# svohr/mixemt

Measured on AMD Instinct MI355X. Metric: read x hap cells/sec through the EM iteration (EM iters/sec reported beside it as em_iters_per_s), 1000000 reads x 5408 haps in total, whole job, higher is better.
Workload: dtype f64

## Files before the change

include/mixemt_hip_tuning.h:

```cpp
#ifndef MIXEMT_HIP_TUNING_H
#define MIXEMT_HIP_TUNING_H

#include <stddef.h>
#include <stdint.h>

#ifdef __cplusplus
extern "C" {
#endif

struct mxm_em_state;

int mxm_reset_tuning(void);

int mxm_set_timing_events(void *ev_start, void *ev_stop);

int mxm_describe_stream_kernel(int32_t H, int32_t nb, char *buf, size_t len);

int mxm_diag_stream_read(const void *src, size_t bytes, int32_t wg_per_cu, int32_t blocked,
                         void *sink, void *stream);

struct mxm_coded;
int mxm_diag_stream_coded(const struct mxm_coded *c, int32_t H, int32_t wg_per_cu, void *sink, void *stream);

int mxm_diag_stream_quads(const struct mxm_coded *c, int32_t H, int32_t wg_per_cu, void *sink, void *stream);

int mxm_set_progress_callback(void (*fn)(const struct mxm_em_state *state_host, int32_t B, void *user),
                              void *user, int32_t every);

int mxm_set_loop_graph(int32_t mode);

int mxm_set_loop_fused(int32_t mode, int32_t chunk);

int mxm_set_fused_coded_grid(int32_t nwg);

int mxm_set_quad_left_grid(int32_t nwg);

int mxm_set_sparse_long_rows(int32_t on);
int mxm_set_sparse_long_entries(int32_t n);

int mxm_set_quad_encoder(int32_t kind);

int mxm_set_coded_batch_tile(int32_t bt);

int mxm_diag_fused_force_abort(int32_t on);

int mxm_diag_fused_stamps(const void *ws, unsigned long long *out_host);

int mxm_set_batch_tile(int32_t bt);

int mxm_set_compact_restarts(int32_t mode);

#define MXM_SAMPLES_TILE_ROWS 32
int mxm_samples_tile_rows(void);

int mxm_set_min_rows_per_wg(int32_t n);

int mxm_set_sparse_max_distinct(int32_t n);

#ifdef __cplusplus
}
#endif
#endif
```

mixemt_amd/_lib.py:

```python

import ctypes
import os

_PKG = os.path.dirname(os.path.abspath(__file__))
LIB_PATH = os.environ.get("MXM_LIB") or os.path.join(_PKG, "lib", "libmixemt_hip.so")

c_i32, c_i64, c_f64 = ctypes.c_int32, ctypes.c_int64, ctypes.c_double
c_ptr, c_size = ctypes.c_void_p, ctypes.c_size_t


class EmState(ctypes.Structure):
    _fields_ = [("done", c_i32), ("iters", c_i32), ("l1", c_f64), ("ticket", ctypes.c_uint32), ("error", ctypes.c_uint32)]


class Coded(ctypes.Structure):
    _fields_ = [("rec", c_ptr), ("rec_off", c_ptr), ("ndist", c_ptr), ("R", c_i64),
                ("P_rest", c_ptr), ("ldp_rest", c_i64), ("w_rest", c_ptr), ("R_rest", c_i64),
                ("wide_rows", c_ptr), ("n_wide", c_i64),
                ("qrec", c_ptr), ("qoff", c_ptr), ("nquad", c_ptr), ("quad_rows", c_ptr), ("n_quad_rows", c_i64),
                ("byte_rows", c_ptr), ("n_byte_rows", c_i64)]


class SampleTile(ctypes.Structure):
    _fields_ = [("sample", c_i32), ("count", c_i32), ("first", c_i64)]
# ... 110 lines not shown
                                      ctypes.POINTER(c_ptr)]),
    "mxm_aln_sizes_of": (ctypes.c_int, [c_ptr, ctypes.POINTER(AlnSizes)]),
    "mxm_aln_fetch": (ctypes.c_int, [c_ptr, c_ptr, c_ptr, c_ptr, c_ptr, c_ptr, c_ptr, c_ptr, c_ptr, c_ptr]),
    "mxm_aln_fetch_fragments": (ctypes.c_int, [c_ptr, c_ptr, c_ptr, c_ptr, c_ptr]),
    "mxm_aln_free": (None, [c_ptr]),
    "mxm_bam_read": (ctypes.c_int, [ctypes.c_char_p, c_i32, ctypes.POINTER(c_ptr)]),
    "mxm_bam_sizes_of": (ctypes.c_int, [c_ptr, ctypes.POINTER(BamSizes)]),
    "mxm_bam_columns": (ctypes.c_int, [c_ptr, ctypes.POINTER(AlnColumns)]),
    "mxm_bam_fetch_names": (ctypes.c_int, [c_ptr, c_ptr, c_ptr, c_ptr, c_ptr]),
    "mxm_bam_free": (None, [c_ptr]),
    "mxm_observe_bases": (ctypes.c_int, [ctypes.POINTER(AlnColumns), c_ptr, c_i32, c_i32, c_i64, c_ptr, c_ptr]),
    "mxm_observe_bases_labelled": (ctypes.c_int, [ctypes.POINTER(AlnColumns), c_ptr, c_ptr, c_i32, c_i32, c_i32, c_i64,
                                                  c_ptr, c_ptr]),
    "mxm_consensus": (ctypes.c_int, [c_ptr, c_i32, c_i64, c_i64, c_i64, c_i32, c_ptr, c_ptr, c_ptr, c_ptr]),
    "mxm_new_variants": (ctypes.c_int, [c_ptr, c_i64, c_i32, ctypes.POINTER(c_i32), c_i32, c_i64, c_ptr, c_ptr, c_ptr]),
    "mxm_first_observed": (ctypes.c_int, [ctypes.POINTER(AlnColumns), c_ptr, c_ptr, c_i32, c_i32, c_i32, c_i64, c_ptr,
                                          c_ptr, c_ptr]),
    "mxm_extend_assign": (ctypes.c_int, [ctypes.POINTER(AlnColumns), c_ptr, c_ptr, c_i32, c_i32, ctypes.POINTER(c_i32),
                                         c_i32, c_i32, c_i32, c_i32, c_ptr, c_i64, c_ptr, c_ptr, c_ptr, c_ptr]),
    "mxm_set_compact_restarts": (ctypes.c_int, [c_i32]),
    "mxm_set_loop_graph": (ctypes.c_int, [c_i32]),
    "mxm_set_loop_fused": (ctypes.c_int, [c_i32, c_i32]),
    "mxm_set_progress_callback": (ctypes.c_int, [c_ptr, c_ptr, c_i32]),
    "mxm_set_min_rows_per_wg": (ctypes.c_int, [c_i32]),
    "mxm_reset_tuning": (ctypes.c_int, []),
    "mxm_describe_stream_kernel": (ctypes.c_int, [c_i32, c_i32, ctypes.c_char_p, c_size]),
    "mxm_set_sparse_max_distinct": (ctypes.c_int, [c_i32]),
    "mxm_row_argmax_votes": (ctypes.c_int, [c_ptr, c_i64, c_ptr, c_i64, c_i32, c_ptr, c_ptr,
                                            c_ptr, c_size, c_ptr]),
    "mxm_first_seen": (ctypes.c_int, [c_ptr, c_i64, c_i32, c_ptr, c_ptr]),
    "mxm_gather_columns": (ctypes.c_int, [c_ptr, c_i64, c_i64, c_i32, c_ptr, c_i32, c_ptr, c_i64, c_ptr]),
    "mxm_fold_logaddexp": (ctypes.c_int, [c_ptr, c_i64, ctypes.POINTER(c_ptr), ctypes.POINTER(c_i64), c_i32,
                                          c_i64, c_i32, c_f64, c_ptr]),
}

FINISH_SIGNATURES = {
    "mxm_samples_finish_workspace_bytes": (c_size, [c_i64, c_i32, c_i32]),
    "mxm_votes_samples": (ctypes.c_int, [ctypes.POINTER(Coded), c_ptr, c_i32, c_i32, c_ptr, c_ptr, c_ptr, c_ptr, c_ptr, c_ptr,
                                         c_ptr, c_ptr, c_ptr, c_ptr, c_ptr, c_size, c_ptr]),
    "mxm_gather_columns_samples": (ctypes.c_int, [ctypes.POINTER(Coded), c_ptr, c_i32, c_i32, c_ptr, c_ptr, c_i32, c_ptr,
                                                  c_ptr, c_size, c_ptr]),
    "mxm_em_loop_samples_narrow": (ctypes.c_int, [ctypes.POINTER(Coded), c_ptr, c_i32, c_i32, c_ptr, c_i32, c_ptr, c_ptr,
                                                  c_ptr, c_ptr, c_ptr, c_ptr, c_f64, c_i32, c_i32, c_ptr, c_ptr, c_size,
                                                  c_ptr, ctypes.POINTER(EmState)]),
    "mxm_assign_reads_samples": (ctypes.c_int, [ctypes.POINTER(Coded), c_ptr, c_i32, c_i32, c_ptr, c_i32, c_ptr, c_ptr,
                                                c_ptr, c_ptr, c_ptr, c_ptr, c_f64, c_ptr, c_ptr, c_ptr, c_size, c_ptr]),
}

VARCHECK_SIGNATURES = {
    "mxm_check_variants_samples": (ctypes.c_int, [c_ptr, c_i32, c_i64, c_ptr, c_ptr, c_i32, c_ptr, c_ptr, c_i32, c_i64, c_ptr,
                                                  c_ptr, c_i32, c_f64, c_f64, c_f64, c_i32, c_i32, c_ptr, c_ptr, c_ptr, c_ptr]),
}

ABI_VERSION = 603

PROGRESS_FN = ctypes.CFUNCTYPE(None, ctypes.POINTER(EmState), c_i32, c_ptr)

_lib = None


class MixemtHipError(RuntimeError):
    pass


def load():
    global _lib
    if _lib is not None:
        return _lib
    if not os.path.exists(LIB_PATH):
        raise MixemtHipError(
            "libmixemt_hip.so is not built (%s); run `python -m mixemt_amd.build` -- "
            "there is no CPU fallback for the EM hot path" % LIB_PATH)
    from . import _dev
    lib = ctypes.CDLL(LIB_PATH)
    try:
        lib.mxm_version.restype = ctypes.c_int
        lib.mxm_version.argtypes = []
        have = lib.mxm_version()
    except AttributeError:
        have = None
    if have != ABI_VERSION:
        raise MixemtHipError("%s reports ABI version %s, this binding was written for %d: rebuild with "
                             "`python -m mixemt_amd.build --force`" % (LIB_PATH, have, ABI_VERSION))
    for name, (restype, argtypes) in (list(SIGNATURES.items()) + list(FINISH_SIGNATURES.items())
                                      + list(VARCHECK_SIGNATURES.items())):
        try:
            fn = getattr(lib, name)
        except AttributeError:
            raise MixemtHipError("%s has ABI version %d but lacks %s: rebuild with "
                                 "`python -m mixemt_amd.build --force`" % (LIB_PATH, have, name))
        fn.restype = restype
        fn.argtypes = argtypes
    _lib = lib
    try:
        if _dev.torch is not None and _dev.torch.cuda.is_available():
            lib.mxm_preload()
    except Exception:
        pass
    return lib


def check(rc, what):
    if rc != 0:
        msg = load().mxm_last_error().decode("utf-8", "replace")
        raise ValueError("%s failed (%d): %s" % (what, rc, msg))
```

mixemt_amd/build.py:

```python

import hashlib
import os
import shutil
import subprocess
import sys

_PKG = os.path.dirname(os.path.abspath(__file__))
_ROOT = os.path.dirname(_PKG)
SRC = os.path.join(_PKG, "csrc", "mixemt_hip.hip")
HDRS = [os.path.join(_ROOT, "include", name) for name in ("mixemt_hip.h", "mixemt_hip_tuning.h", "mixemt_hip_samples_finish.h",
                                                           "mixemt_hip_var_check.h")]
LIB_DIR = os.path.join(_PKG, "lib")
LIB = os.path.join(LIB_DIR, "libmixemt_hip.so")
ARCH = "gfx950"


def _hipcc():
    for cand in (os.environ.get("HIPCC"), shutil.which("hipcc"), "/opt/rocm/bin/hipcc"):
        if cand and os.path.exists(cand):
            return cand
    raise RuntimeError("hipcc not found (set HIPCC or add /opt/rocm/bin to PATH)")


def _sources():
    csrc = os.path.dirname(SRC)
    return sorted(os.path.join(csrc, f) for f in os.listdir(csrc) if f.endswith((".hip", ".hpp"))) + HDRS


def _digest(flags):
    h = hashlib.sha256()
    for path in _sources():
        with open(path, "rb") as fin:
            h.update(fin.read())
    h.update(" ".join(flags).encode())
    return h.hexdigest()


def build(force=False, defines=(), verbose=False, out=None):
    global LIB
    if out is not None:
        LIB = os.path.abspath(out)
    flags = ["--offload-arch=%s" % ARCH, "-O3", "-std=c++17", "-shared", "-fPIC", "-Werror=format",
             "-I" + os.path.join(_ROOT, "include"), "-I" + os.path.dirname(SRC)]
    flags += ["-D%s" % d for d in defines]
    stamp = LIB + ".stamp"
    want = _digest(flags)
    if not force and os.path.exists(LIB) and os.path.exists(stamp):
        with open(stamp) as fin:
            if fin.read().strip() == want:
                return LIB
    os.makedirs(os.path.dirname(LIB), exist_ok=True)
    cmd = [_hipcc()] + flags + [SRC, "-o", LIB, "-lz"]
    if verbose:
        sys.stderr.write(" ".join(cmd) + "\n")
    proc = subprocess.run(cmd, stdout=subprocess.PIPE, stderr=subprocess.STDOUT, text=True)
    if proc.returncode != 0:
        raise RuntimeError("hipcc failed:\n" + proc.stdout)
    with open(stamp, "w") as fout:
        fout.write(want + "\n")
    return LIB


if __name__ == "__main__":
    defs = []
# ... 14 lines not shown
```

mixemt_amd/csrc/coded_kernels.hpp:

```cpp
#ifndef MIXEMT_CODED_KERNELS_HPP
#define MIXEMT_CODED_KERNELS_HPP

#define ENC_THREADS 256
#define ENC_SLOTS 1024
#define ENC_MAX_CODES 256
#define ENC_MAX_WIDE 1024
#define ENC_WIDE_SLOTS 4096
#define ENC_EMPTY 0xFFFFFFFFFFFFFFFFull

__host__ __device__ __forceinline__ int rec_code_bytes(int nd, int ldc) { return nd > ENC_MAX_CODES ? 2 * ldc : ldc; }
__device__ __forceinline__ int rec_code_at(const uint8_t *codes, int h, bool wide) {
    return wide ? (int)reinterpret_cast<const uint16_t *>(codes)[h] : (int)codes[h];
}

template <int NCH, bool WIDE>
__device__ __forceinline__ void encode_one_row(int64_t r, const double *__restrict__ M, int64_t ldm, int H, int ldc,
                                               uint8_t *__restrict__ rec, int64_t rec_cap, int64_t *__restrict__ rec_off,
                                               int32_t *__restrict__ ndist, double *__restrict__ rowmax,
                                               unsigned long long *__restrict__ stats) {
    constexpr int NW = ENC_THREADS / 64;
    constexpr int SLOTS = WIDE ? ENC_WIDE_SLOTS : ENC_SLOTS;
    constexpr int MAXC = WIDE ? ENC_MAX_WIDE : ENC_MAX_CODES;
    constexpr int SPT = SLOTS / ENC_THREADS;
    __shared__ unsigned long long s_key[SLOTS];
// ... 150 lines not shown
                } else {
                    reinterpret_cast<unsigned int *>(rec + off)[t + k * ENC_THREADS] =
                        cd[0] | (cd[1] << 8) | (cd[2] << 16) | (cd[3] << 24);
                }
            }
        }
    }
    if (t == 0) {
        if constexpr (WIDE) {
            if (off >= 0) {
                ndist[r] = D;
                rec_off[r] = off;
                atomicAdd(&stats[1], ~0ull);
            }
        } else {
            rowmax[r] = shift;
            ndist[r] = (off >= 0) ? D : 0;
            rec_off[r] = (off >= 0) ? off : 0;
            if (off < 0) atomicAdd(&stats[1], 1ull);
        }
    }
    __syncthreads();
}

template <int NCH>
__global__ __launch_bounds__(ENC_THREADS) void encode_rows_kernel(
    const double *__restrict__ M, int64_t ldm, int64_t R, int H, int ldc, uint8_t *__restrict__ rec, int64_t rec_cap,
    int64_t *__restrict__ rec_off, int32_t *__restrict__ ndist, double *__restrict__ rowmax,
    unsigned long long *__restrict__ stats) {
    for (int64_t r = blockIdx.x; r < R; r += gridDim.x)
        encode_one_row<NCH, false>(r, M, ldm, H, ldc, rec, rec_cap, rec_off, ndist, rowmax, stats);
}

template <int NCH>
__global__ __launch_bounds__(ENC_THREADS) void encode_wide_rows_kernel(
    const double *__restrict__ M, int64_t ldm, int64_t R, int H, int ldc, uint8_t *__restrict__ rec, int64_t rec_cap,
    int64_t *__restrict__ rec_off, int32_t *__restrict__ ndist, double *__restrict__ rowmax,
    unsigned long long *__restrict__ stats) {
    constexpr int CH = 32;
    __shared__ int s_list[CH];
    __shared__ int s_nlist;
    const int t = threadIdx.x;
    const int64_t nchunk = (R + CH - 1) / CH;
    for (int64_t c = blockIdx.x; c < nchunk; c += gridDim.x) {
        if (t == 0) s_nlist = 0;
        __syncthreads();
        const int64_t r = c * CH + t;
        if (t < CH && r < R && ndist[r] == 0) s_list[atomicAdd(&s_nlist, 1)] = t;
        __syncthreads();
        const int n = s_nlist;
        for (int i = 0; i < n; ++i)
            encode_one_row<NCH, true>(c * CH + s_list[i], M, ldm, H, ldc, rec, rec_cap, rec_off, ndist, rowmax, stats);
        __syncthreads();
    }
}

template <int THREADS, int NCH, int NBUF, bool NT, bool RESIDENT, bool WIDE_PREFETCH, bool CHECK = false>
__device__ __forceinline__ void coded_row_pass(const uint8_t *__restrict__ rec, const int64_t *__restrict__ rec_off,
                                               const int32_t *__restrict__ ndist, int ldc, const double *__restrict__ w,
                                               const int64_t *__restrict__ wide_rows, int64_t n_wide, int64_t R,
                                               const double (&p)[NCH][4], double (&acc)[NCH][4], bool &meta_ready,
                                               int *chk_result = nullptr, const int64_t *__restrict__ row_list = nullptr,
                                               int64_t n_list = 0, const int32_t *__restrict__ nquad = nullptr, int vbid = -1,
                                               int vgrid = 0) {
    static_assert(NBUF >= 3, "codes NBUF - 1 rows ahead, tables NBUF - 2");
    constexpr int NW = THREADS / 64;
    constexpr int AUX = NT ? 2 : 0;
    __shared__ double s_tbl[NBUF][ENC_MAX_CODES];
    __shared__ __attribute__((aligned(16))) double red[NBUF][NW];
    const int t = threadIdx.x, lane = t & 63, wv = t >> 6;
    const int nword = ldc >> 2;
    const int64_t bid = vbid >= 0 ? (int64_t)vbid : (int64_t)blockIdx.x, grid = vbid >= 0 ? (int64_t)vgrid : (int64_t)gridDim.x;
    const row_deal deal(row_list != nullptr ? n_list : R, bid, grid);
    const int voff = t * 4;
    int last_w = t + (NCH - 1) * THREADS;
    if (last_w > nword - 1) last_w = nword - 1;
    const int voff_last = last_w * 4;
    const bool tbl_thread = (THREADS <= ENC_MAX_CODES) || t < ENC_MAX_CODES;
    const int tslot = t & (ENC_MAX_CODES - 1);
    typedef unsigned int u2v __attribute__((ext_vector_type(2)));
    __shared__ int s_chk[2];
    if constexpr (CHECK) {
        if (t == 0) s_chk[0] = s_chk[1] = 0;
        __syncthreads();
    }
    auto list_row = [&](int64_t e) -> int64_t {
        int64_t r = wide_rows[e];
        if constexpr (CHECK) {
            if (r < 0 || r >= R || (e > 0 && wide_rows[e - 1] >= r)) {
                s_chk[1] = 1;
                r = -1;
            }
        }
        return r;
    };
    auto list_nd = [&](int64_t r) -> int {
        if (r < 0) return 0;
        int nd = ndist[r];
        if constexpr (CHECK) {
            if (nd <= ENC_MAX_CODES) {
                s_chk[1] = 1;
                nd = 0;
            }
        }
        return nd;
    };
// ... 443 lines not shown
```

mixemt_amd/csrc/mixemt_hip.hip:

```cpp
#include <hip/hip_runtime.h>
#include <stdint.h>
#include <stdio.h>
#include <stdlib.h>
#include <string.h>
#include <math.h>
#include <algorithm>
#include <atomic>
#include <mutex>
#include <type_traits>
#include <utility>
#include <vector>

#include "mixemt_hip.h"
#include "mixemt_hip_tuning.h"

#include "common.hpp"
#include "aln_encode.hpp"
#include "bam_reader.hpp"
#include "coded_kernels.hpp"
#include "quad_kernels.hpp"
#include "quad_batched_kernels.hpp"
#include "build_kernels.hpp"
#include "build_lut_kernels.hpp"
#include "build_sparse_kernels.hpp"
#include "em_kernels.hpp"
#include "estep_kernels.hpp"
#include "aux_kernels.hpp"
#include "records_kernels.hpp"
#include "fused_kernels.hpp"
#include "fused_cols_kernels.hpp"
#include "fused_coded_kernels.hpp"
#include "fused_narrow_kernels.hpp"
#include "samples_kernels.hpp"
#include "samples_finish_kernels.hpp"
#include "exchange.hpp"
#include "aln_walk.hpp"
#include "observe_kernels.hpp"
#include "var_check_kernels.hpp"
#include "assemble_kernels.hpp"


struct mxm_em_state;
typedef void (*mxm_progress_fn)(const mxm_em_state *state_host, int32_t B, void *user);
struct mxm_tuning {
    int sparse_maxd = -1;
    int min_rows_per_wg = 8;
    int compact_restarts = 2;
    int max_bt = 4;
    int loop_graph = -1;
    int loop_fused = -1;
    int fused_chunk = 0;
    int fused_cols = 1;
    int fused_coded_wg = 0;
    int quad_left_wg = 0;
    int sparse_long_entries = 5120;
    int quad_encoder = 1;
    int sparse_long = 1;
    int coded_bt = 3;
    int fused_force_abort = 0;
    double fused_cells = 1.0e8;
    hipEvent_t ev_start = nullptr, ev_stop = nullptr;
    mxm_progress_fn progress = nullptr;
    void *progress_user = nullptr;
    int progress_every = 10;
};
static std::mutex g_tune_mu;
static mxm_tuning g_tune;
static thread_local mxm_tuning T;
#define MXM_ENTER() do { std::lock_guard<std::mutex> lk_(g_tune_mu); T = g_tune; } while (0)
template <typename F>
static int tune_set(F f) {
    std::lock_guard<std::mutex> lk(g_tune_mu);
    f(g_tune);
    return 0;
}
extern "C" int mxm_reset_tuning(void) {
    return tune_set([](mxm_tuning &t) { t = mxm_tuning(); });
}

static inline int clamp_grid(int64_t want, int cap) {
    if (want < 1) want = 1;
    return (int)(want < cap ? want : cap);
}

static inline int64_t part_ld(int H) { return ((int64_t)H + 1) & ~(int64_t)1; }

static hipError_t raise_dynamic_lds(const void *kernel, size_t bytes, const char *name) {
    const hipError_t e = hipFuncSetAttribute(kernel, hipFuncAttributeMaxDynamicSharedMemorySize, (int)bytes);
    if (e != hipSuccess)
        snprintf(g_err, sizeof(g_err), "%s: cannot opt into %zu bytes of dynamic LDS: %s", name, bytes,
                 hipGetErrorString(e));
    return e;
}
static int dynamic_lds_ok(const void *kernel, size_t bytes, const char *name, const char *who = nullptr, int H = 0,
                          const char *too_wide = nullptr) {
    if (too_wide != nullptr && bytes > 150 * 1024) return fail(-1, "%s: H=%d %s", who, H, too_wide);
    if (bytes > 60 * 1024 && raise_dynamic_lds(kernel, bytes, name) != hipSuccess) return -2;
    return 0;
}

#define RC_TRY(expr)                                                                         \
    do {                                                                                     \
        const int rc_ = (expr);                                                              \
        if (rc_ != 0) return rc_;                                                            \
    } while (0)

template <int MAX, typename F>
static bool dispatch_width(int n, F &&f) {
    if constexpr (MAX < 1) {
// ... 286 lines not shown
extern "C" int mxm_linearize(const double *M, int64_t ldm, int64_t R, int32_t H, double *P, int64_t ldp,
                             double *rowmax, void *stream) {
    if (R < 0 || H <= 0) return fail(-1, "mxm_linearize: bad shape");
    if (ldm < H || ldp < H || (ldp & 1)) return fail(-1, "mxm_linearize: ldp must be even and >= H (ldp=%lld)", (long long)ldp);
    if (R == 0) return 0;
    if (wide_rows_ok(M, ldm, H) && (reinterpret_cast<uintptr_t>(P) & 15) == 0 &&
        linearize_wide<double>(M, ldm, R, (int)H, P, ldp, rowmax, (hipStream_t)stream) == 0) {
        HIP_TRY(hipGetLastError());
        return 0;
    }
    const int grid = clamp_grid(R, num_cu() * 8);
    hipLaunchKernelGGL(linearize_kernel, dim3(grid), dim3(ROW_THREADS), 0, (hipStream_t)stream, M, ldm, R,
                       (int)H, P, ldp, rowmax);
    HIP_TRY(hipGetLastError());
    return 0;
}

extern "C" int mxm_set_timing_events(void *ev_start, void *ev_stop) {
    return tune_set([=](mxm_tuning &t) { t.ev_start = (hipEvent_t)ev_start; t.ev_stop = (hipEvent_t)ev_stop; });
}

extern "C" int mxm_set_min_rows_per_wg(int32_t n) {
    if (n < 1) return fail(-1, "mxm_set_min_rows_per_wg: n < 1");
    return tune_set([n](mxm_tuning &t) { t.min_rows_per_wg = n; });
}

extern "C" int mxm_set_compact_restarts(int32_t mode) {
    return tune_set([mode](mxm_tuning &t) { t.compact_restarts = mode < 0 ? 0 : (mode > 2 ? 2 : mode); });
}

extern "C" int mxm_set_batch_tile(int32_t bt) {
    if (bt < 1 || bt > 4) return fail(-1, "mxm_set_batch_tile: tile must be 1..4");
    return tune_set([bt](mxm_tuning &t) { t.max_bt = bt; });
}

extern "C" int mxm_set_fused_coded_grid(int32_t nwg) {
    return tune_set([nwg](mxm_tuning &t) { t.fused_coded_wg = nwg > 0 ? nwg : 0; });
}

extern "C" int mxm_set_sparse_long_rows(int32_t on) {
    return tune_set([on](mxm_tuning &t) { t.sparse_long = on ? 1 : 0; });
}
extern "C" int mxm_set_sparse_long_entries(int32_t n) {
    return tune_set([n](mxm_tuning &t) { t.sparse_long_entries = n > 0 ? n : 0; });
}
extern "C" int mxm_set_coded_batch_tile(int32_t bt) {
    if (bt != 1 && bt != 3) return fail(-1, "mxm_set_coded_batch_tile: 1 or 3, got %d", bt);
    return tune_set([bt](mxm_tuning &t) { t.coded_bt = bt; });
}
extern "C" int mxm_set_quad_encoder(int32_t kind) {
    if (kind != 0 && kind != 1) return fail(-1, "mxm_set_quad_encoder: 0 or 1, got %d", kind);
    return tune_set([kind](mxm_tuning &t) { t.quad_encoder = kind; });
}
extern "C" int mxm_set_quad_left_grid(int32_t nwg) {
    return tune_set([nwg](mxm_tuning &t) { t.quad_left_wg = nwg > 0 ? nwg : 0; });
}

extern "C" int mxm_diag_fused_force_abort(int32_t on) {
    return tune_set([on](mxm_tuning &t) { t.fused_force_abort = on ? 1 : 0; });
}

#ifndef MXM_V1_THREADS
#define MXM_V1_THREADS 256
#endif
#ifndef MXM_V1_NBUF
#define MXM_V1_NBUF 2
#endif
#ifndef MXM_V1_WG_PER_CU
#define MXM_V1_WG_PER_CU 2
#endif
#ifndef MXM_V2_THREADS
#define MXM_V2_THREADS 512
#endif
#ifndef MXM_V2_NBUF
#define MXM_V2_NBUF 2
#endif
#ifndef MXM_V3_THREADS
#define MXM_V3_THREADS 512
#endif
#ifndef MXM_V3_NBUF
#define MXM_V3_NBUF 2
#endif
#ifndef MXM_V4_THREADS
#define MXM_V4_THREADS 512
#endif
#ifndef MXM_V4_NBUF
#define MXM_V4_NBUF 2
#endif
#ifndef MXM_V2_PREG
#define MXM_V2_PREG 1
#endif
#ifndef MXM_V3_PREG
#define MXM_V3_PREG 2
#endif
#ifndef MXM_V4_PREG
#define MXM_V4_PREG 2
#endif
#ifndef MXM_V1B_THREADS
#define MXM_V1B_THREADS 512
#endif
#ifndef MXM_V1B_NBUF
#define MXM_V1B_NBUF 3
#endif
#define MXM_MAX_COL2 4096
#define MXM_LDS_BUDGET (156 * 1024)

// ... 238 lines not shown
    for (int b = 0; b < B;) {
        const int left = B - b;
        const int passes = (left + max_bt - 1) / max_bt;
        const int nb = (left + passes - 1) / passes;
        const mxm_em_state *st = state ? state + b : nullptr;
        int rc;
        if (linear)
            rc = em_iter_linear_tile(P, ldp, w, props, R, (int)H, nb, slots_from(b), state, colsum, (double *)ws,
                                     (hipStream_t)stream, b == 0);
        else
            rc = em_iter_log_one(M, ldm, w, ln_props ? ln_props + (int64_t)b * H : nullptr, R, (int)H, st,
                                 colsum + (int64_t)b * H, (double *)ws, (hipStream_t)stream);
        if (rc != 0) return rc;
        b += nb;
    }
    return 0;
}

extern "C" int mxm_linearize_f32(const double *M, int64_t ldm, int64_t R, int32_t H, float *P, int64_t ldp,
                                 double *rowmax, void *stream) {
    if (R < 0 || H <= 0) return fail(-1, "mxm_linearize_f32: bad shape");
    if (ldm < H || ldp < H || (ldp & 3)) return fail(-1, "mxm_linearize_f32: ldp must be a multiple of 4 and >= H (ldp=%lld)", (long long)ldp);
    if (R == 0) return 0;
    if (wide_rows_ok(M, ldm, H) && (reinterpret_cast<uintptr_t>(P) & 7) == 0 && (ldp & 1) == 0 &&
        linearize_wide<float>(M, ldm, R, (int)H, P, ldp, rowmax, (hipStream_t)stream) == 0) {
        HIP_TRY(hipGetLastError());
        return 0;
    }
    const int grid = clamp_grid(R, num_cu() * 8);
    hipLaunchKernelGGL(linearize_f32_kernel, dim3(grid), dim3(ROW_THREADS), 0, (hipStream_t)stream, M, ldm, R, (int)H,
                       P, ldp, rowmax);
    HIP_TRY(hipGetLastError());
    return 0;
}

extern "C" int mxm_em_iter_f32(const float *P, int64_t ldp, const double *w, const double *props, int64_t R,
                               int32_t H, int32_t B, const mxm_em_state *state, double *colsum, void *ws,
                               size_t ws_bytes, void *stream) {
    MXM_ENTER();
    if (R <= 0 || H <= 0 || B <= 0) return fail(-1, "mxm_em_iter_f32: bad shape R=%lld H=%d", (long long)R, H);
    if (!mxm_linear_supported(H)) return fail(-1, "mxm_em_iter_f32: H=%d outside the linear kernel's range", H);
    if (P == nullptr || (ldp & 3) || ldp < H) return fail(-1, "mxm_em_iter_f32: ldp must be a multiple of 4 and >= H");
    if (ws == nullptr || ws_bytes < mxm_workspace_bytes(R, H, B)) return fail(-1, "mxm_em_iter_f32: workspace too small");
    for (int b = 0; b < B; ++b) {
        const int rc = em_iter_f32_one(P, ldp, w, props + (int64_t)b * H, R, (int)H, state ? state + b : nullptr,
                                       colsum + (int64_t)b * H, (double *)ws, (hipStream_t)stream, b == 0);
        if (rc != 0) return rc;
    }
    return 0;
}

extern "C" size_t mxm_coded_bytes(int64_t R, int32_t H) { return mxm_record_bytes(R, H); }

extern "C" int mxm_encode_rows(const double *M, int64_t ldm, int64_t R, int32_t H, uint8_t *rec, size_t rec_bytes,
                               int64_t *rec_off, int32_t *ndist, double *rowmax, int64_t *stats, void *stream) {
    if (R <= 0 || H <= 0 || ldm < H) return fail(-1, "mxm_encode_rows: bad shape R=%lld H=%d", (long long)R, H);
    if (!mxm_linear_supported(H) || (reinterpret_cast<uintptr_t>(M) & 7) != 0)
        return fail(-1, "mxm_encode_rows: needs H in [65, 8192] (H=%d ldm=%lld)", H, (long long)ldm);
    if (rec == nullptr || (reinterpret_cast<uintptr_t>(rec) & 15) || rec_bytes < (size_t)coded_ld(H) + 16 * ENC_MAX_CODES)
        return fail(-1, "mxm_encode_rows: record buffer missing, unaligned or smaller than one record");
    if (rec_off == nullptr || ndist == nullptr || rowmax == nullptr || stats == nullptr)
        return fail(-1, "mxm_encode_rows: output arrays required");
    hipStream_t s = (hipStream_t)stream;
    HIP_TRY(hipMemsetAsync(stats, 0, 2 * sizeof(int64_t), s));
    const int ldc = coded_ld(H);
    const int nch = (ldc / 4 + ENC_THREADS - 1) / ENC_THREADS;
    const int grid = clamp_grid(R, num_cu() * 4);
    const int grid_w = clamp_grid((R + 31) / 32, num_cu() * 3);
    const bool ok = dispatch_width<8>(nch, [&](auto n) {
        constexpr int NCH = decltype(n)::value;
        unsigned long long *st = reinterpret_cast<unsigned long long *>(stats);
        hipLaunchKernelGGL((encode_rows_kernel<NCH>), dim3(grid), dim3(ENC_THREADS), 0, s, M, ldm, R, (int)H, ldc, rec,
                           (int64_t)rec_bytes, rec_off, ndist, rowmax, st);
        hipLaunchKernelGGL((encode_wide_rows_kernel<NCH>), dim3(grid_w), dim3(ENC_THREADS), 0, s, M, ldm, R, (int)H, ldc, rec,
                           (int64_t)rec_bytes, rec_off, ndist, rowmax, st);
    });
    if (!ok) return fail(-1, "mxm_encode_rows: H=%d outside the kernel's range", H);
    HIP_TRY(hipGetLastError());
    return 0;
}

static int coded_check(const mxm_coded *c, int32_t H, const char *who) {
    if (c == nullptr || c->R <= 0 || H <= 0 || !mxm_linear_supported(H))
        return fail(-1, "%s: bad coded matrix (rows %lld, H %d)", who, (long long)(c ? c->R : 0), H);
    if (c->rec == nullptr || c->rec_off == nullptr || c->ndist == nullptr) return fail(-1, "%s: coded matrix arrays missing", who);
    if (c->R_rest < 0 || (c->R_rest > 0 && (c->P_rest == nullptr || c->ldp_rest < H || (c->ldp_rest & 1) ||
                                            (reinterpret_cast<uintptr_t>(c->P_rest) & 15))))
        return fail(-1, "%s: the dense rest needs 16-byte aligned rows with an even ld >= H", who);
    if (c->n_wide < 0 || (c->n_wide > 0 && c->wide_rows == nullptr)) return fail(-1, "%s: n_wide > 0 needs wide_rows", who);
    if (c->qrec != nullptr) {
        if (c->qoff == nullptr || c->nquad == nullptr || c->n_quad_rows < 0 || c->n_byte_rows < 0 ||
            (c->n_quad_rows > 0 && c->quad_rows == nullptr) || (c->n_byte_rows > 0 && c->byte_rows == nullptr) ||
            (reinterpret_cast<uintptr_t>(c->qrec) & 31))
            return fail(-1, "%s: quad dictionary arrays missing (or qrec not 32-byte aligned)", who);
        if (c->n_quad_rows + c->n_byte_rows + c->n_wide + c->R_rest != c->R)
            return fail(-1, "%s: quad_rows + byte_rows + wide_rows + the dense rest must be all %lld rows", who, (long long)c->R);
    }
    return 0;
}

static int rest_check(const char *who, int32_t H, const double *M_rest, int64_t ldm_rest, const int64_t *rest_rows, int64_t n_rest) {
    if (n_rest < 0 || (n_rest > 0 && (M_rest == nullptr || rest_rows == nullptr || ldm_rest < H)))
        return fail(-1, "%s: the rows without a record need M_rest, rest_rows and ldm_rest >= H", who);
    return 0;
}

extern "C" size_t mxm_quad_bytes(int64_t R, int32_t H) {
    (void)H;
    constexpr size_t largest = QUAD_CODE_BYTES + QUAD_MAX * 32, per_piece = (size_t)QUAD_CHUNK / largest;
    return R > 0 ? (((size_t)R + per_piece - 1) / per_piece + 5120) * (size_t)QUAD_CHUNK : 0;
}

extern "C" int mxm_expand_tables(const uint8_t *maj, const int32_t *mk_ptr, const uint16_t *mk_hap, const uint8_t *mk_base,
                                 const uint8_t *map256, int32_t S, int32_t H, int64_t lde, uint8_t *out, void *stream) {
    if (maj == nullptr || mk_ptr == nullptr || mk_hap == nullptr || mk_base == nullptr || out == nullptr || S <= 0 || H <= 0 || lde < H)
        return fail(-1, "mxm_expand_tables: bad arguments");
    hipLaunchKernelGGL(expand_tables_kernel, dim3(clamp_grid(S, num_cu() * 8)), dim3(256), 0, (hipStream_t)stream, maj, mk_ptr, mk_hap,
                       mk_base, map256, (int)S, (int)H, lde, out);
    HIP_TRY(hipGetLastError());
    return 0;
}

extern "C" size_t mxm_quad_lists_scratch_bytes(int64_t R) {
    return R > 0 ? (size_t)((R + QLIST_CHUNK - 1) / QLIST_CHUNK) * 2 * sizeof(long long) : 0;
}

extern "C" int mxm_quad_lists(const int32_t *ndist, const int32_t *nquad, int64_t R, int64_t *quad_rows, int64_t *byte_rows,
                              int64_t *counts, void *scratch, size_t scratch_bytes, void *stream) {
// ... 1701 lines not shown
```

Measured before the change: 875.1 billion.

## Add prefetching row encoder that loads the next row while encoding the current one

Adds new row-encoding kernels in which each workgroup issues buffer loads for its next row while it dedups and encodes the current row. Distinct values are queued per wave through ballot compaction, so only one insertion per distinct key reaches the shared hash table. Grid size now comes from the occupancy query, and the new path is on by default through a row_encoder tuning switch. This aims to hide global-memory latency in the encode stage, at the cost of more registers and LDS and a more intricate synchronisation scheme.

Result: no change. 878.9 billion (median of 4 runs) (+0.4%).

```diff
diff --git a/include/mixemt_hip_row_encoder.h b/include/mixemt_hip_row_encoder.h
--- /dev/null
+++ b/include/mixemt_hip_row_encoder.h
@@ -0,0 +1,15 @@
+#ifndef MIXEMT_HIP_ROW_ENCODER_H
+#define MIXEMT_HIP_ROW_ENCODER_H
+
+#include <stdint.h>
+
+#ifdef __cplusplus
+extern "C" {
+#endif
+
+int mxm_set_row_encoder(int32_t kind);
+
+#ifdef __cplusplus
+}
+#endif
+#endif
diff --git a/include/mixemt_hip_tuning.h b/include/mixemt_hip_tuning.h
--- a/include/mixemt_hip_tuning.h
+++ b/include/mixemt_hip_tuning.h
@@ -40,6 +40,8 @@
 
 int mxm_set_quad_encoder(int32_t kind);
 
+#include "mixemt_hip_row_encoder.h"
+
 int mxm_set_coded_batch_tile(int32_t bt);
 
 int mxm_diag_fused_force_abort(int32_t on);
diff --git a/mixemt_amd/_lib.py b/mixemt_amd/_lib.py
--- a/mixemt_amd/_lib.py
+++ b/mixemt_amd/_lib.py
@@ -186,6 +186,10 @@
                                                   c_ptr, c_i32, c_f64, c_f64, c_f64, c_i32, c_i32, c_ptr, c_ptr, c_ptr, c_ptr]),
 }
 
+ROW_ENCODER_SIGNATURES = {
+    "mxm_set_row_encoder": (ctypes.c_int, [c_i32]),
+}
+
 ABI_VERSION = 603
 
 PROGRESS_FN = ctypes.CFUNCTYPE(None, ctypes.POINTER(EmState), c_i32, c_ptr)
@@ -217,7 +221,7 @@
         raise MixemtHipError("%s reports ABI version %s, this binding was written for %d: rebuild with "
                              "`python -m mixemt_amd.build --force`" % (LIB_PATH, have, ABI_VERSION))
     for name, (restype, argtypes) in (list(SIGNATURES.items()) + list(FINISH_SIGNATURES.items())
-                                      + list(VARCHECK_SIGNATURES.items())):
+                                      + list(VARCHECK_SIGNATURES.items()) + list(ROW_ENCODER_SIGNATURES.items())):
         try:
             fn = getattr(lib, name)
         except AttributeError:
diff --git a/mixemt_amd/build.py b/mixemt_amd/build.py
--- a/mixemt_amd/build.py
+++ b/mixemt_amd/build.py
@@ -9,7 +9,7 @@
 _ROOT = os.path.dirname(_PKG)
 SRC = os.path.join(_PKG, "csrc", "mixemt_hip.hip")
 HDRS = [os.path.join(_ROOT, "include", name) for name in ("mixemt_hip.h", "mixemt_hip_tuning.h", "mixemt_hip_samples_finish.h",
-                                                           "mixemt_hip_var_check.h")]
+                                                           "mixemt_hip_var_check.h", "mixemt_hip_row_encoder.h")]
 LIB_DIR = os.path.join(_PKG, "lib")
 LIB = os.path.join(LIB_DIR, "libmixemt_hip.so")
 ARCH = "gfx950"
diff --git a/mixemt_amd/csrc/coded_kernels.hpp b/mixemt_amd/csrc/coded_kernels.hpp
--- a/mixemt_amd/csrc/coded_kernels.hpp
+++ b/mixemt_amd/csrc/coded_kernels.hpp
@@ -226,6 +226,338 @@
         for (int i = 0; i < n; ++i)
             encode_one_row<NCH, true>(c * CH + s_list[i], M, ldm, H, ldc, rec, rec_cap, rec_off, ndist, rowmax, stats);
         __syncthreads();
+    }
+}
+
+#define ENC_QCAP 512
+
+struct enc_source {
+    __amdgpu_buffer_rsrc_t rsrc;
+    const double *last;
+};
+__device__ __forceinline__ enc_source enc_row_source(const double *__restrict__ M, int64_t ldm, int64_t r, bool live, int H) {
+    const double *row = M + (live ? r : 0) * ldm;
+    return {__builtin_amdgcn_make_buffer_rsrc(const_cast<double *>(row), 0, live ? H * 8 : 0, 0x00020000),
+            ((H & 1) && live) ? row + (H - 1) : nullptr};
+}
+template <int NCH>
+__device__ __forceinline__ void enc_issue_chunk(const enc_source &src, double (&x)[NCH][4], int k) {
+    typedef unsigned int u4 __attribute__((ext_vector_type(4)));
+    const int off = ((int)threadIdx.x + k * ENC_THREADS) * 32;
+    const d2 a = __builtin_bit_cast(d2, (u4)__builtin_amdgcn_raw_buffer_load_b128(src.rsrc, off, 0, 2));
+    const d2 b = __builtin_bit_cast(d2, (u4)__builtin_amdgcn_raw_buffer_load_b128(src.rsrc, off, 16, 2));
+    x[k][0] = a.x;
+    x[k][1] = a.y;
+    x[k][2] = b.x;
+    x[k][3] = b.y;
+}
+template <int NCH>
+__device__ __forceinline__ void enc_patch_tail(double (&x)[NCH][4], double tail, int H) {
+    if (H & 1) {
+        const int t = threadIdx.x;
+#pragma unroll
+        for (int k = 0; k < NCH; ++k) {
+            if (4 * (t + k * ENC_THREADS) == H - 1) x[k][0] = tail;
+            if (4 * (t + k * ENC_THREADS) + 2 == H - 1) x[k][2] = tail;
+        }
+    }
+}
+__device__ __forceinline__ void enc_wave_fence() {
+    __builtin_amdgcn_fence(__ATOMIC_RELEASE, "wavefront");
+    __builtin_amdgcn_wave_barrier();
+    __builtin_amdgcn_fence(__ATOMIC_ACQUIRE, "wavefront");
+}
+
+template <bool WIDE>
+struct enc_lds {
+    static constexpr int SLOTS = WIDE ? ENC_WIDE_SLOTS : ENC_SLOTS;
+    static constexpr int MAXC = WIDE ? ENC_MAX_WIDE : ENC_MAX_CODES;
+    unsigned long long key[SLOTS];
+    unsigned long long q[ENC_THREADS / 64][ENC_QCAP];
+    unsigned short code[SLOTS];
+    unsigned short inv[MAXC];
+    double red[ENC_THREADS / 64];
+    int wcnt[ENC_THREADS / 64];
+    int flag, n;
+    long long off;
+};
+template <bool WIDE>
+__device__ __forceinline__ void enc_clear(enc_lds<WIDE> &S) {
+    for (int i = threadIdx.x; i < enc_lds<WIDE>::SLOTS; i += ENC_THREADS) S.key[i] = ENC_EMPTY;
+    if (threadIdx.x == 0) {
+        S.flag = 0;
+        S.n = 0;
+    }
+    __syncthreads();
+}
+
+template <int NCH, bool WIDE>
+__device__ __forceinline__ void encode_row_ahead(enc_lds<WIDE> &S, double (&x)[NCH][4], double &tail, int64_t r,
+                                                 const enc_source &next, const double *__restrict__ M, int64_t ldm, int H,
+                                                 int ldc, uint8_t *__restrict__ rec, int64_t rec_cap,
+                                                 int64_t *__restrict__ rec_off, int32_t *__restrict__ ndist,
+                                                 double *__restrict__ rowmax, unsigned long long *__restrict__ stats) {
+    constexpr int NW = ENC_THREADS / 64;
+    constexpr int SLOTS = enc_lds<WIDE>::SLOTS;
+    constexpr int MAXC = enc_lds<WIDE>::MAXC;
+    constexpr int SPT = SLOTS / ENC_THREADS;
+    const int t = threadIdx.x, lane = t & 63, wv = t >> 6;
+    typedef unsigned int u2 __attribute__((ext_vector_type(2)));
+
+    enc_patch_tail<NCH>(x, tail, H);
+
+    auto probe = [&](unsigned long long key) -> int {
+        unsigned int h = (unsigned int)((key ^ (key >> 29)) * 0x9E3779B97F4A7C15ull >> 40) & (SLOTS - 1);
+        for (int probes = 0;; ++probes) {
+            const unsigned long long old = atomicCAS(&S.key[h], ENC_EMPTY, key);
+            if (old == ENC_EMPTY) {
+                if (atomicAdd(&S.n, 1) >= MAXC) S.flag = 1;
+                break;
+            }
+            if (old == key) break;
+            h = (h + 1) & (SLOTS - 1);
+            if (probes >= SLOTS) {
+                S.flag = 1;
+                break;
+            }
+        }
+        return (int)h;
+    };
+    auto given_up = [&]() { return __hip_atomic_load(&S.flag, __ATOMIC_RELAXED, __HIP_MEMORY_SCOPE_WORKGROUP) != 0; };
+
+    const bool wave_live = 256 * wv < H;
+    const unsigned long long wkey = (unsigned long long)__double_as_longlong(readlane_f64(x[0][0], 0));
+    if (wave_live && lane == 0) S.q[wv][0] = wkey;
+    int qn = __builtin_amdgcn_readfirstlane(wave_live ? 1 : 0);
+    int ref[NCH][4];
+    unsigned long long prev_key = wkey;
+    int prev_ref = 0;
+#pragma unroll
+    for (int k = 0; k < NCH; ++k) {
+        if (qn + 4 * 64 <= ENC_QCAP) {
+#pragma unroll
+            for (int e = 0; e < 4; ++e) {
+                const bool valid = (k < NCH - 1) || 4 * (t + k * ENC_THREADS) + e < H;
+                const unsigned long long key = (unsigned long long)__double_as_longlong(x[k][e]);
+                const bool need = valid && key != wkey && key != prev_key;
+                const unsigned long long votes = __builtin_amdgcn_ballot_w64(need);
+                const int pos = qn + (int)__builtin_amdgcn_mbcnt_hi((unsigned int)(votes >> 32),
+                                                                    __builtin_amdgcn_mbcnt_lo((unsigned int)votes, 0u));
+                if (need) S.q[wv][pos] = key;
+                const int rf = need ? pos : (key == wkey ? 0 : prev_ref);
+                qn += __builtin_popcountll(votes);
+                ref[k][e] = rf;
+                if (valid) {
+                    prev_key = key;
+                    prev_ref = rf;
+                }
+            }
+        } else {
+            const bool give_up = given_up();
+#pragma unroll
+            for (int e = 0; e < 4; ++e) {
+                const bool valid = (k < NCH - 1) || 4 * (t + k * ENC_THREADS) + e < H;
+                const unsigned long long key = (unsigned long long)__double_as_longlong(x[k][e]);
+                int rf = (key == wkey) ? 0 : prev_ref;
+                if (valid && key != wkey && key != prev_key) {
+                    rf = ENC_QCAP;
+                    if (key == ENC_EMPTY) S.flag = 1;
+                    else if (!give_up) rf = ENC_QCAP + probe(key);
+                }
+                ref[k][e] = rf;
+                if (valid) {
+                    prev_key = key;
+                    prev_ref = rf;
+                }
+            }
+        }
+        enc_issue_chunk<NCH>(next, x, k);
+    }
+    tail = (next.last != nullptr) ? *next.last : 0.0;
+    enc_wave_fence();
+    for (int i = lane; i - lane < qn; i += 64) {
+        if (given_up()) break;
+        if (i < qn) {
+            const unsigned long long key = S.q[wv][i];
+            int sl = 0;
+            if (key == ENC_EMPTY) S.flag = 1;
+            else sl = probe(key);
+            S.q[wv][i] = (unsigned long long)sl;
+        }
+    }
+    __syncthreads();
+    const bool dense = (S.flag != 0);
+    const int cbytes = WIDE ? 2 * ldc : ldc;
+    long long off_mine = -1, end_mine = 0;
+    {
+        const int n_keys = S.n;
+        const int64_t bytes = (int64_t)cbytes + 16 * (int64_t)n_keys;
+        if (t == 0 && !dense && n_keys <= MAXC && (!WIDE || n_keys > ENC_MAX_CODES)) {
+            int zero = 0;
+            asm volatile("" : "+v"(zero));
+            off_mine = (long long)atomicAdd(&stats[zero], (unsigned long long)bytes);
+            end_mine = bytes;
+        }
+    }
+
+    int cnt = 0;
+    double m = -INFINITY;
+#pragma unroll
+    for (int j = 0; j < SPT; ++j) {
+        const unsigned long long kk = S.key[SPT * t + j];
+        if (kk != ENC_EMPTY) {
+            ++cnt;
+            m = fmax(m, __longlong_as_double((long long)kk));
+        }
+    }
+    const int incl = wave_inclusive_scan_i32(cnt);
+    if (lane == 63) S.wcnt[wv] = incl;
+    if (!WIDE && dense) {
+        const double *row = M + r * ldm;
+        m = -INFINITY;
+        for (int h = t; h < H; h += ENC_THREADS) m = fmax(m, row[h]);
+    }
+    m = wave_max_lane63(m);
+    if (lane == 63) S.red[wv] = m;
+    __syncthreads();
+    m = fmax(fmax(S.red[0], S.red[1]), fmax(S.red[2], S.red[3]));
+    const double shift = isfinite(m) ? m : 0.0;
+    int base = 0, D = 0;
+#pragma unroll
+    for (int q = 0; q < NW; ++q) {
+        if (q < wv) base += S.wcnt[q];
+        D += S.wcnt[q];
+    }
+    int code = base + incl - cnt;
+#pragma unroll
+    for (int j = 0; j < SPT; ++j) {
+        if (S.key[SPT * t + j] != ENC_EMPTY) {
+            if (code < MAXC) S.inv[code] = (unsigned short)(SPT * t + j);
+            S.code[SPT * t + j] = (unsigned short)code++;
+        }
+    }
+    if (t == 0) S.off = (off_mine + end_mine > rec_cap) ? -1 : off_mine;
+    __syncthreads();
+    const long long off = S.off;
+    if (off >= 0) {
+#pragma unroll
+        for (int k = 0; k < NCH; ++k) {
+            const int c0 = 4 * (t + k * ENC_THREADS);
+            if (c0 < ldc) {
+                unsigned int cd[4];
+#pragma unroll
+                for (int e = 0; e < 4; ++e) {
+                    const int rf = ref[k][e];
+                    const int queued = *reinterpret_cast<const int *>(&S.q[wv][rf & (ENC_QCAP - 1)]);
+                    const int sl = (rf >= ENC_QCAP ? rf - ENC_QCAP : queued) & (SLOTS - 1);
+                    cd[e] = (c0 + e < H) ? (unsigned int)S.code[sl] : 0u;
+                }
+                if constexpr (WIDE) {
+                    u2 word;
+                    word.x = cd[0] | (cd[1] << 16);
+                    word.y = cd[2] | (cd[3] << 16);
+                    reinterpret_cast<u2 *>(rec + off)[t + k * ENC_THREADS] = word;
+                } else {
+                    reinterpret_cast<unsigned int *>(rec + off)[t + k * ENC_THREADS] =
+                        cd[0] | (cd[1] << 8) | (cd[2] << 16) | (cd[3] << 24);
+                }
+            }
+        }
+    }
+    if (D <= MAXC) {
+        double *tbl = reinterpret_cast<double *>(rec + off + cbytes);
+        for (int c = t; c < D; c += ENC_THREADS) {
+            const int sl = S.inv[c];
+            const unsigned long long kk = S.key[sl];
+            S.key[sl] = ENC_EMPTY;
+            if (off >= 0) {
+                const double mval = __longlong_as_double((long long)kk);
+                tbl[c] = exp(mval - shift);
+                tbl[D + c] = mval;
+            }
+        }
+    } else {
+#pragma unroll
+        for (int j = 0; j < SPT; ++j) S.key[SPT * t + j] = ENC_EMPTY;
+    }
+    if (t == 0) {
+        S.flag = 0;
+        S.n = 0;
+        if constexpr (WIDE) {
+            if (off >= 0) {
+                ndist[r] = D;
+                rec_off[r] = off;
+                atomicAdd(&stats[1], ~0ull);
+            }
+        } else {
+            rowmax[r] = shift;
+            ndist[r] = (off >= 0) ? D : 0;
+            rec_off[r] = (off >= 0) ? off : 0;
+            if (off < 0) atomicAdd(&stats[1], 1ull);
+        }
+    }
+    __syncthreads();
+}
+
+template <int NCH>
+__global__ __launch_bounds__(ENC_THREADS) void encode_rows_ahead_kernel(
+    const double *__restrict__ M, int64_t ldm, int64_t R, int H, int ldc, uint8_t *__restrict__ rec, int64_t rec_cap,
+    int64_t *__restrict__ rec_off, int32_t *__restrict__ ndist, double *__restrict__ rowmax,
+    unsigned long long *__restrict__ stats) {
+    __shared__ enc_lds<false> S;
+    enc_clear(S);
+    double x[NCH][4];
+    const enc_source first = enc_row_source(M, ldm, blockIdx.x, blockIdx.x < R, H);
+#pragma unroll
+    for (int k = 0; k < NCH; ++k) enc_issue_chunk<NCH>(first, x, k);
+    double tail = (first.last != nullptr) ? *first.last : 0.0;
+    for (int64_t r = blockIdx.x; r < R; r += gridDim.x) {
+        const int64_t rn = r + gridDim.x;
+        encode_row_ahead<NCH, false>(S, x, tail, r, enc_row_source(M, ldm, rn, rn < R, H), M, ldm, H, ldc, rec, rec_cap,
+                                     rec_off, ndist, rowmax, stats);
+    }
+}
+
+template <int NCH>
+__global__ __launch_bounds__(ENC_THREADS) void encode_wide_rows_ahead_kernel(
+    const double *__restrict__ M, int64_t ldm, int64_t R, int H, int ldc, uint8_t *__restrict__ rec, int64_t rec_cap,
+    int64_t *__restrict__ rec_off, int32_t *__restrict__ ndist, double *__restrict__ rowmax,
+    unsigned long long *__restrict__ stats) {
+    constexpr int CH = 32;
+    __shared__ enc_lds<true> S;
+    __shared__ int s_list[CH];
+    __shared__ int s_nlist;
+    const int t = threadIdx.x;
+    const int64_t nchunk = (R + CH - 1) / CH;
+    int64_t c = (int64_t)blockIdx.x - (int64_t)gridDim.x;
+    int i = 0, n = 0;
+    auto next_row = [&]() -> int64_t {
+        for (;;) {
+            if (i < n) return c * CH + __builtin_amdgcn_readfirstlane(s_list[i++]);
+            c += gridDim.x;
+            if (c >= nchunk) return -1;
+            __syncthreads();
+            if (t == 0) s_nlist = 0;
+            __syncthreads();
+            const int64_t rr = c * CH + t;
+            if (t < CH && rr < R && ndist[rr] == 0) s_list[atomicAdd(&s_nlist, 1)] = t;
+            __syncthreads();
+            n = __builtin_amdgcn_readfirstlane(s_nlist);
+            i = 0;
+        }
+    };
+    enc_clear(S);
+    double x[NCH][4];
+    int64_t r = next_row();
+    const enc_source first = enc_row_source(M, ldm, r, r >= 0, H);
+#pragma unroll
+    for (int k = 0; k < NCH; ++k) enc_issue_chunk<NCH>(first, x, k);
+    double tail = (first.last != nullptr) ? *first.last : 0.0;
+    while (r >= 0) {
+        const int64_t rn = next_row();
+        encode_row_ahead<NCH, true>(S, x, tail, r, enc_row_source(M, ldm, rn, rn >= 0, H), M, ldm, H, ldc, rec, rec_cap,
+                                    rec_off, ndist, rowmax, stats);
+        r = rn;
     }
 }
 
diff --git a/mixemt_amd/csrc/mixemt_hip.hip b/mixemt_amd/csrc/mixemt_hip.hip
--- a/mixemt_amd/csrc/mixemt_hip.hip
+++ b/mixemt_amd/csrc/mixemt_hip.hip
@@ -55,6 +55,7 @@
     int quad_left_wg = 0;
     int sparse_long_entries = 5120;
     int quad_encoder = 1;
+    int row_encoder = 1;
     int sparse_long = 1;
     int coded_bt = 3;
     int fused_force_abort = 0;
@@ -447,6 +448,10 @@
     if (kind != 0 && kind != 1) return fail(-1, "mxm_set_quad_encoder: 0 or 1, got %d", kind);
     return tune_set([kind](mxm_tuning &t) { t.quad_encoder = kind; });
 }
+extern "C" int mxm_set_row_encoder(int32_t kind) {
+    if (kind != 0 && kind != 1) return fail(-1, "mxm_set_row_encoder: 0 or 1, got %d", kind);
+    return tune_set([kind](mxm_tuning &t) { t.row_encoder = kind; });
+}
 extern "C" int mxm_set_quad_left_grid(int32_t nwg) {
     return tune_set([nwg](mxm_tuning &t) { t.quad_left_wg = nwg > 0 ? nwg : 0; });
 }
@@ -791,8 +796,26 @@
 
 extern "C" size_t mxm_coded_bytes(int64_t R, int32_t H) { return mxm_record_bytes(R, H); }
 
+template <typename K>
+static int enc_grid(K kernel, int64_t want) {
+    int per_cu = 0;
+    if (hipOccupancyMaxActiveBlocksPerMultiprocessor(&per_cu, kernel, ENC_THREADS, 0) != hipSuccess || per_cu < 1) per_cu = 2;
+    return clamp_grid(want, num_cu() * per_cu);
+}
+template <int NCH>
+static void launch_rows_ahead(hipStream_t s, const double *M, int64_t ldm, int64_t R, int H, int ldc, uint8_t *rec, int64_t rec_bytes,
+                              int64_t *rec_off, int32_t *ndist, double *rowmax, unsigned long long *st) {
+    const auto first = encode_rows_ahead_kernel<NCH>;
+    const auto second = encode_wide_rows_ahead_kernel<NCH>;
+    hipLaunchKernelGGL(first, dim3(enc_grid(first, R)), dim3(ENC_THREADS), 0, s, M, ldm, R, H, ldc, rec, rec_bytes, rec_off, ndist,
+                       rowmax, st);
+    hipLaunchKernelGGL(second, dim3(enc_grid(second, (R + 31) / 32)), dim3(ENC_THREADS), 0, s, M, ldm, R, H, ldc, rec, rec_bytes,
+                       rec_off, ndist, rowmax, st);
+}
+
 extern "C" int mxm_encode_rows(const double *M, int64_t ldm, int64_t R, int32_t H, uint8_t *rec, size_t rec_bytes,
                                int64_t *rec_off, int32_t *ndist, double *rowmax, int64_t *stats, void *stream) {
+    MXM_ENTER();
     if (R <= 0 || H <= 0 || ldm < H) return fail(-1, "mxm_encode_rows: bad shape R=%lld H=%d", (long long)R, H);
     if (!mxm_linear_supported(H) || (reinterpret_cast<uintptr_t>(M) & 7) != 0)
         return fail(-1, "mxm_encode_rows: needs H in [65, 8192] (H=%d ldm=%lld)", H, (long long)ldm);
@@ -806,13 +829,17 @@
     const int nch = (ldc / 4 + ENC_THREADS - 1) / ENC_THREADS;
     const int grid = clamp_grid(R, num_cu() * 4);
     const int grid_w = clamp_grid((R + 31) / 32, num_cu() * 3);
+    const int kind = T.row_encoder;
     const bool ok = dispatch_width<8>(nch, [&](auto n) {
         constexpr int NCH = decltype(n)::value;
         unsigned long long *st = reinterpret_cast<unsigned long long *>(stats);
-        hipLaunchKernelGGL((encode_rows_kernel<NCH>), dim3(grid), dim3(ENC_THREADS), 0, s, M, ldm, R, (int)H, ldc, rec,
-                           (int64_t)rec_bytes, rec_off, ndist, rowmax, st);
-        hipLaunchKernelGGL((encode_wide_rows_kernel<NCH>), dim3(grid_w), dim3(ENC_THREADS), 0, s, M, ldm, R, (int)H, ldc, rec,
-                           (int64_t)rec_bytes, rec_off, ndist, rowmax, st);
+        if (kind == 0) {
+            hipLaunchKernelGGL((encode_rows_kernel<NCH>), dim3(grid), dim3(ENC_THREADS), 0, s, M, ldm, R, (int)H, ldc, rec,
+                               (int64_t)rec_bytes, rec_off, ndist, rowmax, st);
+            hipLaunchKernelGGL((encode_wide_rows_kernel<NCH>), dim3(grid_w), dim3(ENC_THREADS), 0, s, M, ldm, R, (int)H, ldc, rec,
+                               (int64_t)rec_bytes, rec_off, ndist, rowmax, st);
+        }
+        else launch_rows_ahead<NCH>(s, M, ldm, R, (int)H, ldc, rec, (int64_t)rec_bytes, rec_off, ndist, rowmax, st);
     });
     if (!ok) return fail(-1, "mxm_encode_rows: H=%d outside the kernel's range", H);
     HIP_TRY(hipGetLastError());
```
